# lenskit/csr

Measured on AMD Instinct MI355X. Metric: spmv_gflops, higher is better.
Workload: dtype f64

## Files before the change

### csr_amd/csrc/acc_groups.h

```cpp
#pragma once
#include <algorithm>
#include <cstdint>
#include <numeric>
#include <vector>

namespace csrk {
namespace accgroups {

constexpr int MAX_GROUPS = 3;
constexpr int XCDS = 8;

struct Deal {
    std::vector<std::vector<int32_t>> groups;
    std::vector<int32_t> first;
};

inline Deal deal_rows(const int64_t *lens, int32_t n, int G, int32_t cap)
{
    Deal d;
    d.first.push_back(0);
    if (n <= 0) return d;
    if (cap < 1) cap = 1;
    if (G < 1) G = 1;
    if (G > MAX_GROUPS) G = MAX_GROUPS;
    if (G == 1) {
        for (int32_t g0 = 0; g0 < n; g0 += cap) {
            const int32_t g1 = n - g0 < cap ? n : g0 + cap;
            std::vector<int32_t> g((size_t)(g1 - g0));
            std::iota(g.begin(), g.end(), g0);
            d.groups.push_back(std::move(g));
            d.first.push_back((int32_t)d.groups.size());
        }
        return d;
    }
    std::vector<int32_t> rank((size_t)n);
    std::iota(rank.begin(), rank.end(), 0);
    std::stable_sort(rank.begin(), rank.end(), [&](int32_t a, int32_t b) { return lens[a] > lens[b]; });
    const int64_t per_launch = (int64_t)G * cap;
    for (int64_t r0 = 0; r0 < n; r0 += per_launch) {
        const int64_t nl = n - r0 < per_launch ? n - r0 : per_launch;
        const int gb = (int)std::min<int64_t>(G, (nl + cap - 1) / cap);
        const size_t base = d.groups.size();
        d.groups.resize(base + (size_t)gb);
        for (int64_t i = 0; i < nl; i++) d.groups[base + (size_t)(i % gb)].push_back(rank[(size_t)(r0 + i)]);
        for (int g = 0; g < gb; g++) std::sort(d.groups[base + (size_t)g].begin(), d.groups[base + (size_t)g].end());
        d.first.push_back((int32_t)d.groups.size());
    }
    return d;
}

constexpr int64_t TILE_ENTRIES = 512;
constexpr int64_t MIN_SEG_TILES = 48;
inline int choose_groups(const int64_t *lens, int32_t n, int g_max, int32_t cap, int64_t floor_len, int64_t nb, int32_t cus)
{
    if (cap < 1) cap = 1;
    if (g_max > MAX_GROUPS) g_max = MAX_GROUPS;
    if (g_max < 2 || n <= cap) return 1;
    std::vector<int64_t> sl;
    for (int32_t i = 0; i < n; i++)
        if (lens[i] >= floor_len) sl.push_back(lens[i]);
    for (int g = g_max; g > 1; g--) {
        const int64_t k = std::min<int64_t>((int64_t)sl.size(), (int64_t)g * cap);
        if (k <= (int64_t)(g - 1) * cap) continue;
        if (k < (int64_t)sl.size()) std::nth_element(sl.begin(), sl.begin() + k, sl.end(), [](int64_t a, int64_t b) { return a > b; });
        int64_t entries = 0;
        for (int64_t i = 0; i < k; i++) entries += sl[(size_t)i];
        if (entries / TILE_ENTRIES >= MIN_SEG_TILES * ((int64_t)g * nb + cus)) return g;
    }
    return 1;
}

constexpr int64_t NIB_MIN_WG_TILES = 16;
inline bool choose_nib(int knob, int64_t launch_entries, int32_t launch_wgs)
{
    if (knob >= 0) return knob != 0;
    if (launch_wgs < 1) launch_wgs = 1;
    return launch_entries >= 0 && launch_entries / TILE_ENTRIES >= NIB_MIN_WG_TILES * (int64_t)launch_wgs;
}

inline int32_t group_wgs(int32_t cus, int gb, int g)
{
    const int32_t n = cus / gb + (g < cus % gb ? 1 : 0);
    return n < 1 ? 1 : n;
}

inline std::vector<uint32_t> place_wgs(const int32_t *n_wg, int gb)
{
    int64_t total = 0;
    int32_t w_max = 0;
    for (int g = 0; g < gb; g++) {
        total += n_wg[g];
        w_max = std::max(w_max, n_wg[g]);
    }
    std::vector<uint32_t> map((size_t)total, ~0u);
    int64_t fill[XCDS], room[XCDS];
    for (int c = 0; c < XCDS; c++) {
        fill[c] = 0;
        room[c] = total / XCDS + (c < total % XCDS ? 1 : 0);
    }
    std::vector<uint32_t> late;
    for (int32_t w = 0; w < w_max; w++)
        for (int g = 0; g < gb; g++) {
            if (w >= n_wg[g]) continue;
            const uint32_t id = ((uint32_t)g << 16) | (uint32_t)w;
            const int c = w % XCDS;
            if (fill[c] < room[c]) map[(size_t)(c + XCDS * fill[c]++)] = id;
            else late.push_back(id);
        }
    size_t b = 0;
    for (uint32_t id : late) {
        while (map[b] != ~0u) b++;
        map[b] = id;
    }
    return map;
}

}
}
```

### csr_amd/csrc/spmv_plan.hip

```cpp
#include "spmv_plan.h"

#include <algorithm>
#include <cstring>
#include <ctime>
#include <type_traits>

namespace csrk {
struct PlanTrace {
    bool on;
    double t0;
    static double now()
    {
        timespec ts;
        clock_gettime(CLOCK_MONOTONIC, &ts);
        return ts.tv_sec * 1e3 + ts.tv_nsec * 1e-6;
    }
    PlanTrace() : on(getenv("CSRK_PLAN_TRACE") != nullptr), t0(0.0)
    {
        if (on) {
            (void)hipDeviceSynchronize();
            t0 = now();
        }
    }
    void lap(const char *what)
    {
        if (!on) return;
        (void)hipDeviceSynchronize();
        const double t = now();
        fprintf(stderr, "[csrk plan] %-28s %8.3f ms\n", what, t - t0);
        t0 = t;
    }
};

template <class P>
__global__ void merge_plan_kernel(const P *__restrict__ rp, int32_t nrows, int64_t nnz, int items,
                                  int64_t n_tiles, int32_t *__restrict__ tile_row)
{
    int64_t t = (int64_t)blockIdx.x * blockDim.x + threadIdx.x;
    if (t > n_tiles) return;
    int64_t total = (int64_t)nrows + nnz;
    int64_t d = t * items;
    if (d > total) d = total;
    int64_t lo = d - nnz > 0 ? d - nnz : 0;
    int64_t hi = d < nrows ? d : nrows;
    while (lo < hi) {
        int64_t mid = (lo + hi) >> 1;
        if ((int64_t)rp[mid + 1] <= d - mid - 1)
            lo = mid + 1;
        else
            hi = mid;
    }
    tile_row[t] = (int32_t)lo;
}

constexpr int HOT_TABLE = 8192, HOT_PROBE = 4;
constexpr int HOT_THREADS = 512;
template <class P>
__global__ __launch_bounds__(HOT_THREADS) void hot_count_kernel(const P *__restrict__ rp, const P *__restrict__ rp_light,
                                                               const int32_t *__restrict__ ci, int32_t nrows, int64_t row_stride,
                                                               int32_t *__restrict__ cnt, unsigned long long *__restrict__ total)
{
    __shared__ int32_t s_key[HOT_TABLE];
    __shared__ int32_t s_cnt[HOT_TABLE];
    __shared__ int32_t s_start[HOT_THREADS / WAVE][WAVE];
    for (int k = threadIdx.x; k < HOT_TABLE; k += HOT_THREADS) {
        s_key[k] = -1;
        s_cnt[k] = 0;
    }
    __syncthreads();
    const int lane = threadIdx.x & (WAVE - 1), wv = threadIdx.x / WAVE;
    int32_t *starts = s_start[wv];
    const int64_t n_groups = ((int64_t)nrows + WAVE * row_stride - 1) / (WAVE * row_stride);
    unsigned long long n = 0;
    for (int64_t q = (int64_t)blockIdx.x * (HOT_THREADS / WAVE) + wv; q < n_groups; q += (int64_t)gridDim.x * (HOT_THREADS / WAVE)) {
        const int64_t r = q * WAVE * row_stride + lane;
        int64_t s = 0;
        int32_t len = 0;
        if (r < nrows && !(rp_light && rp_light[r + 1] == rp_light[r])) {
            s = rp[r];
            const int64_t l = (int64_t)rp[r + 1] - s;
            len = (int32_t)(l > 128 ? 128 : l);
        }
        const int32_t start = wave_exscan_i32(len, lane);
        const int32_t all = __builtin_amdgcn_readlane(start + len, WAVE - 1);
        __builtin_amdgcn_wave_barrier();
        starts[lane] = start;
        __builtin_amdgcn_wave_barrier();
        for (int32_t d0 = 0; d0 < all; d0 += WAVE) {
            const int32_t d = d0 + lane;
            const bool in = d < all;
            int p = 0;
#pragma unroll
            for (int step = WAVE / 2; step; step >>= 1)
                if (in && starts[p + step] <= d) p += step;
            const int64_t k = __shfl(s, p, WAVE) + (d - __shfl(start, p, WAVE));
            if (!in) continue;
            const int32_t c = ci[k];
            uint32_t slot = ((uint32_t)c * 2654435761u) >> 19;
            bool done = false;
#pragma unroll
            for (int pr = 0; pr < HOT_PROBE && !done; pr++) {
                const int32_t old = atomicCAS(&s_key[slot], -1, c);
                if (old == -1 || old == c) {
                    atomicAdd(&s_cnt[slot], 1);
                    done = true;
                }
                slot = (slot + 1) & (HOT_TABLE - 1);
            }
            if (!done) atomicAdd(&cnt[c], 1);
        }
        if (lane == 0) n += (unsigned long long)all;
    }
    __syncthreads();
    for (int k = threadIdx.x; k < HOT_TABLE; k += HOT_THREADS)
        if (s_key[k] >= 0) atomicAdd(&cnt[s_key[k]], s_cnt[k]);
    for (int off = WAVE / 2; off; off >>= 1) n += __shfl_down(n, off, WAVE);
    if ((threadIdx.x & (WAVE - 1)) == 0 && n) atomicAdd(total, n);
}

__global__ __launch_bounds__(256) void hot_census_kernel(const int32_t *__restrict__ cnt, int32_t ncols, int32_t thr,
                                                        unsigned long long *__restrict__ out)
{
    unsigned long long n = 0, sum = 0;
    for (int64_t c = (int64_t)blockIdx.x * 256 + threadIdx.x; c < ncols; c += (int64_t)gridDim.x * 256) {
        const int32_t v = cnt[c];
        if (v >= thr) {
            n++;
            sum += (unsigned long long)v;
        }
    }
    for (int off = WAVE / 2; off; off >>= 1) {
        n += __shfl_down(n, off, WAVE);
        sum += __shfl_down(sum, off, WAVE);
    }
    if ((threadIdx.x & (WAVE - 1)) == 0 && n) {
        atomicAdd(&out[0], n);
        atomicAdd(&out[1], sum);
    }
}

constexpr int HOT_HIST = 65536, HOT_HIST_LDS = 2048;
__global__ __launch_bounds__(256) void hot_hist_kernel(const int32_t *__restrict__ cnt, int32_t ncols,
                                                      unsigned long long *__restrict__ hist_n,
                                                      unsigned long long *__restrict__ hist_sum)
{
    __shared__ unsigned int s_n[HOT_HIST_LDS];
    for (int k = threadIdx.x; k < HOT_HIST_LDS; k += 256) s_n[k] = 0u;
    __syncthreads();
    for (int64_t c = (int64_t)blockIdx.x * 256 + threadIdx.x; c < ncols; c += (int64_t)gridDim.x * 256) {
        const int32_t v = cnt[c];
        if (v < HOT_HIST_LDS) {
            atomicAdd(&s_n[v], 1u);
        } else {
            const int b = v < HOT_HIST ? v : HOT_HIST;
            atomicAdd(&hist_n[b], 1ull);
            atomicAdd(&hist_sum[b], (unsigned long long)v);
        }
// ... 635 lines not shown

__global__ void vec_fill_kernel(const int64_t *__restrict__ seg_off, int32_t nrows, int32_t *__restrict__ seg_row)
{
    int64_t r = (int64_t)blockIdx.x * blockDim.x + threadIdx.x;
    if (r >= nrows) return;
    for (int64_t q = seg_off[r]; q < seg_off[r + 1]; q++) seg_row[q] = (int32_t)r;
}

constexpr int HEAVY_STREAMS = 8;

template <class P, int VT>
static int build_panel(Matrix *m, Panel *pn, const std::vector<int32_t> &rows, int64_t nnz_rows, int32_t cb,
                       int tpw, bool xcd_streams, hipStream_t s)
{
    PlanTrace tr;
    const P *rp = (const P *)m->d_rowptrs;
    const int32_t n = (int32_t)rows.size();
    const int32_t nb = (int32_t)ceil_div(m->ncols > 0 ? m->ncols : 1, cb);
    const int64_t pairs = (int64_t)n * nb;
    CSRK_TRY(pn->row_list.alloc((size_t)n * 4));
    CSRK_TRY(stage_h2d(pn->row_list.p, rows.data(), (size_t)n * 4, s));
    DevBuf off, bends;
    CSRK_TRY(off.alloc((size_t)(pairs + 1) * 8));
    const unsigned g = (unsigned)xcd_block_chunk_grid(ceil_div(n, 256), nb);
    panel_count_kernel<P><<<g, 256, 0, s>>>(rp, m->d_colinds, pn->row_list.as<int32_t>(), n, nb, cb, off.as<int64_t>());
    CSRK_LAUNCH_CHECK();
    CSRK_TRY(exclusive_scan_i64(off.as<int64_t>(), off.as<int64_t>(), pairs, s));
    pn->p64 = nnz_rows > INT32_MAX;
    CSRK_TRY(pn->rp.alloc((size_t)(pairs + 1) * (pn->p64 ? 8 : 4)));
    CSRK_TRY(pn->ci.alloc((size_t)nnz_rows * 4));
    CSRK_TRY(pn->vs.alloc((size_t)nnz_rows * 8));
    if (pn->p64)
        panel_fill_kernel<P, VT, int64_t><<<g, 256, 0, s>>>(rp, m->d_colinds, m->d_values, pn->row_list.as<int32_t>(), n, nb,
                                                          cb, off.as<int64_t>(), pn->rp.as<int64_t>(),
                                                          pn->ci.as<int32_t>(), pn->vs.as<double>());
    else
        panel_fill_kernel<P, VT, int32_t><<<g, 256, 0, s>>>(rp, m->d_colinds, m->d_values, pn->row_list.as<int32_t>(), n, nb,
                                                          cb, off.as<int64_t>(), pn->rp.as<int32_t>(),
                                                          pn->ci.as<int32_t>(), pn->vs.as<double>());
    CSRK_LAUNCH_CHECK();
    CSRK_TRY(bends.alloc((size_t)(nb + 1) * 8));
    panel_blockends_kernel<<<(unsigned)ceil_div(nb + 1, 256), 256, 0, s>>>(off.as<int64_t>(), n, nb, bends.as<int64_t>());
    CSRK_LAUNCH_CHECK();
    std::vector<int64_t> be((size_t)nb + 1), t0((size_t)nb + 1);
    CSRK_TRY(stage_d2h(be.data(), bends.p, (size_t)(nb + 1) * 8, s));
    CSRK_HIP(hipStreamSynchronize(s));
    t0[0] = 0;
    for (int32_t b = 0; b < nb; b++) t0[b + 1] = t0[b] + ceil_div((int64_t)n + be[b + 1] - be[b], MERGE_ITEMS);
    const int64_t n_tiles = t0[nb];
    CSRK_TRY(stage_h2d(bends.p, t0.data(), (size_t)(nb + 1) * 8, s));
    tr.lap("  tier 1: count, scan, fill");
    CSRK_TRY(pn->tile.alloc((size_t)n_tiles * sizeof(PanelTile)));
    if (pn->p64)
        panel_plan_kernel<int64_t><<<(unsigned)ceil_div(n_tiles, 256), 256, 0, s>>>(
            pn->rp.as<int64_t>(), n, nb, bends.as<int64_t>(), n_tiles, MERGE_ITEMS, pn->tile.as<PanelTile>());
    else
        panel_plan_kernel<int32_t><<<(unsigned)ceil_div(n_tiles, 256), 256, 0, s>>>(
            pn->rp.as<int32_t>(), n, nb, bends.as<int64_t>(), n_tiles, MERGE_ITEMS, pn->tile.as<PanelTile>());
    CSRK_LAUNCH_CHECK();
    CSRK_REQUIRE(((int64_t)cb << PANEL_POS_BITS) <= (1ll << 32), "column block too wide for the tile's index word");
    if (n_tiles > 0) {
        panel_colsort_kernel<<<(unsigned)n_tiles, 256, 0, s>>>(pn->tile.as<PanelTile>(), cb, pn->ci.as<int32_t>(), pn->vs.as<double>());
        CSRK_LAUNCH_CHECK();
    }
    tr.lap("  tier 1: tiles, column order");

    std::vector<PanelGroup> groups;
    auto block_groups = [&](int32_t b, std::vector<PanelGroup> &out) {
        for (int64_t t = t0[b]; t < t0[b + 1]; t += tpw) {
            PanelGroup gq;
            gq.t0 = t;
            gq.nt = (int32_t)(t0[b + 1] - t < tpw ? t0[b + 1] - t : tpw);
            gq.blk = b;
            out.push_back(gq);
        }
    };
    if (!xcd_streams || nb < 2 * HEAVY_STREAMS) {
        for (int32_t b = 0; b < nb; b++) block_groups(b, groups);
    } else {
        std::vector<PanelGroup> st[HEAVY_STREAMS];
        size_t longest = 0;
        for (int32_t b = 0; b < nb; b++) block_groups(b, st[b % HEAVY_STREAMS]);
        for (int q = 0; q < HEAVY_STREAMS; q++) longest = st[q].size() > longest ? st[q].size() : longest;
        PanelGroup pad;
        pad.t0 = 0;
        pad.nt = 0;
        pad.blk = 0;
        groups.reserve(longest * HEAVY_STREAMS);
        for (size_t i = 0; i < longest; i++)
            for (int q = 0; q < HEAVY_STREAMS; q++) groups.push_back(i < st[q].size() ? st[q][i] : pad);
    }
    int32_t ncs = 0;
    {
        std::vector<PanelTile> ht((size_t)n_tiles);
        CSRK_TRY(stage_d2h(ht.data(), pn->tile.p, (size_t)n_tiles * sizeof(PanelTile), nullptr));
        std::vector<int32_t> cnt((size_t)n, 0);
        for (int64_t t = 0; t < n_tiles; t++)
            if ((int64_t)ht[(size_t)t].i1 < pairs) {
                const int32_t c = ++cnt[(size_t)(ht[(size_t)t].i1 % n)];
                ncs = c > ncs ? c : ncs;
            }
        ncs = ncs < PANEL_CARRY_ROWS ? ncs : PANEL_CARRY_ROWS;
        std::vector<int32_t> crp((size_t)n + 1, 0), cidx;
        bool listed = false;
        for (int32_t h = 0; h < n; h++) {
            crp[(size_t)h + 1] = crp[(size_t)h] + (cnt[(size_t)h] > ncs ? cnt[(size_t)h] - ncs : 0);
            listed = listed || cnt[(size_t)h] > ncs;
        }
        cidx.resize((size_t)crp[(size_t)n] + 1);
        pn->listed = crp[(size_t)n];
        std::vector<int32_t> seen((size_t)n, 0);
        for (int64_t t = 0; t < n_tiles; t++) {
            PanelTile &T = ht[(size_t)t];
            T.cslot = -1;
            if ((int64_t)T.i1 >= pairs) continue;
            const int32_t h = (int32_t)(T.i1 % n), j = seen[(size_t)h]++;
            if (j < ncs) T.cslot = pairs + (int64_t)j * n + h;
            else cidx[(size_t)(crp[(size_t)h] + j - ncs)] = (int32_t)t;
        }
        CSRK_TRY(stage_h2d(pn->tile.p, ht.data(), (size_t)n_tiles * sizeof(PanelTile), nullptr));
        if (listed) {
            CSRK_TRY(pn->crp.alloc(crp.size() * 4));
            CSRK_TRY(pn->cidx.alloc(cidx.size() * 4));
            CSRK_TRY(stage_h2d(pn->crp.p, crp.data(), crp.size() * 4, nullptr));
            CSRK_TRY(stage_h2d(pn->cidx.p, cidx.data(), cidx.size() * 4, nullptr));
        }
    }
    pn->groups = (int64_t)groups.size();
    pn->pad_groups = 0;
    for (const PanelGroup &gq : groups) pn->pad_groups += gq.nt == 0;
    CSRK_TRY(pn->group.alloc(groups.size() * sizeof(PanelGroup)));
    CSRK_TRY(stage_h2d(pn->group.p, groups.data(), groups.size() * sizeof(PanelGroup), s));
    CSRK_TRY(pn->carry_row.alloc((size_t)n_tiles * 4));
    CSRK_TRY(pn->carry_val.alloc((size_t)n_tiles * 8));
    CSRK_TRY(pn->y.alloc((size_t)(pairs + (int64_t)ncs * n) * 8));
    if (ncs) {
        std::vector<double> neg0((size_t)ncs * n, -0.0);
        CSRK_TRY(stage_h2d(pn->y.as<double>() + pairs, neg0.data(), neg0.size() * 8, s));
    }
    pn->ncs = ncs;
    CSRK_HIP(hipStreamSynchronize(s));
    tr.lap("  tier 1: groups, carries (host)");
    pn->on = true;
    pn->cb = cb;
    pn->nb = nb;
    pn->nrow = n;
    pn->rows = pairs;
    pn->tiles = n_tiles;
    pn->nnz = nnz_rows;
    return CSRK_OK;
}

enum { ACC_FORM_RAW = 0, ACC_FORM_FIX56 = 1, ACC_FORM_NIB = 2 };
template <class P, int VT>
static int build_acc_panel(Matrix *m, AccPanel *ap, const int32_t *rows, const int64_t *lens, int32_t n, int64_t nnz_rows,
                           hipStream_t s, int32_t wg_want = 0, int form = ACC_FORM_FIX56)
{
    ap->fix56 = false;
    ap->nib = false;
    ap->fx_g = 0;
    const P *rp = (const P *)m->d_rowptrs;
    const int32_t nb = (int32_t)ceil_div(m->ncols > 0 ? m->ncols : 1, ACC_CB);
    PlanTrace tr;
    const int64_t pairs = (int64_t)n * nb;
    CSRK_TRY(ap->row_list.alloc((size_t)n * 4));
    CSRK_TRY(stage_h2d(ap->row_list.p, rows, (size_t)n * 4, s));
    DevBuf off, bends, pstart, d_trow, d_tpiece;
    CSRK_TRY(off.alloc((size_t)(pairs + 1) * 8));
    std::vector<int32_t> trow, tpiece;
    for (int32_t c = 0; c < n; c++)
        for (int64_t pc = 0; pc * ACC_PIECE < lens[c]; pc++) {
            trow.push_back(c);
            tpiece.push_back((int32_t)pc);
        }
    const int64_t n_tasks = (int64_t)trow.size();
    CSRK_TRY(pstart.alloc((size_t)(pairs + n) * 4));
    CSRK_TRY(d_trow.alloc((size_t)(n_tasks ? n_tasks : 1) * 4));
    CSRK_TRY(d_tpiece.alloc((size_t)(n_tasks ? n_tasks : 1) * 4));
    CSRK_TRY(stage_h2d(d_trow.p, trow.data(), (size_t)n_tasks * 4, s));
    CSRK_TRY(stage_h2d(d_tpiece.p, tpiece.data(), (size_t)n_tasks * 4, s));
    acc_pairstart_kernel<P><<<(unsigned)(ceil_div(ceil_div(n_tasks * WAVE, 256), 8) * 8), 256, 0, s>>>(
        rp, m->d_colinds, ap->row_list.as<int32_t>(), n, nb, ACC_CB, d_trow.as<int32_t>(), d_tpiece.as<int32_t>(), n_tasks,
        pstart.as<int32_t>());
    CSRK_LAUNCH_CHECK();
    tr.lap("  tier 0: pair starts");
    acc_paircount_kernel<<<(unsigned)ceil_div(pairs, 256), 256, 0, s>>>(pstart.as<int32_t>(), pairs, n, off.as<int64_t>());
    CSRK_LAUNCH_CHECK();
    DevBuf gap;
    CSRK_TRY(gap.alloc((size_t)pairs * 4));
    acc_gap_kernel<<<(unsigned)ceil_div((int64_t)nb * WAVE, 256), 256, 0, s>>>(off.as<int64_t>(), n, nb, gap.as<int32_t>());
    CSRK_LAUNCH_CHECK();
    CSRK_TRY(exclusive_scan_i64(off.as<int64_t>(), off.as<int64_t>(), pairs, s));
    CSRK_TRY(bends.alloc((size_t)(nb + 1) * 8));
    panel_blockends_kernel<<<(unsigned)ceil_div(nb + 1, 256), 256, 0, s>>>(off.as<int64_t>(), n, nb, bends.as<int64_t>());
    CSRK_LAUNCH_CHECK();
    std::vector<int64_t> be((size_t)nb + 1), t0((size_t)nb + 1);
    CSRK_TRY(stage_d2h(be.data(), bends.p, (size_t)(nb + 1) * 8, s));
    CSRK_HIP(hipStreamSynchronize(s));
    t0[0] = 0;
    for (int32_t b = 0; b < nb; b++) t0[b + 1] = t0[b] + ceil_div(be[b + 1] - be[b], ACC_TILE);
    const int64_t n_tiles = t0[nb];
    CSRK_TRY(stage_h2d(bends.p, t0.data(), (size_t)(nb + 1) * 8, s));
    tr.lap("  tier 0: counts, gaps, scan");
    int cus = 0;
    CSRK_HIP(hipDeviceGetAttribute(&cus, hipDeviceAttributeMultiprocessorCount, m->device));
    int64_t n_wg = wg_want > 0 ? wg_want : cus > 0 ? cus : 256;
    if (n_wg > n_tiles) n_wg = n_tiles;
    if (n_wg < 1) n_wg = 1;
    std::vector<int64_t> wg_t0((size_t)n_wg + 1);
    int64_t share_max = 0;
    for (int64_t w = 0; w <= n_wg; w++) wg_t0[(size_t)w] = n_tiles * w / n_wg;
    for (int64_t w = 0; w < n_wg; w++) share_max = std::max(share_max, wg_t0[(size_t)w + 1] - wg_t0[(size_t)w]);
    const int64_t n_phys = share_max * n_wg;
    DevBuf d_wg_t0;
    CSRK_TRY(d_wg_t0.alloc((size_t)(n_wg + 1) * 8));
    CSRK_TRY(stage_h2d(d_wg_t0.p, wg_t0.data(), (size_t)(n_wg + 1) * 8, s));
    ap->f32 = VT == CSRK_VAL_F32;
    DevBuf fx;
    CSRK_TRY(fx.alloc(16));
    if (VT == CSRK_VAL_F64 && n > 0 && form != ACC_FORM_RAW) {
        const char *env = getenv("CSRK_SPMV_FIX56");
        if (!(env && env[0] == '0')) {
            int32_t h[4] = {0, INT32_MAX, INT32_MIN, 0};
            CSRK_TRY(stage_h2d(fx.p, h, sizeof h, s));
            acc_range_kernel<P><<<dim3((unsigned)n, 16), 256, 0, s>>>(rp, (const double *)m->d_values, ap->row_list.as<int32_t>(),
                                                                     fx.as<int32_t>());
            CSRK_LAUNCH_CHECK();
            CSRK_TRY(stage_d2h(h, fx.p, sizeof h, s));
            CSRK_HIP(hipStreamSynchronize(s));
            fix56::Range r;
            r.bad = h[0];
            r.lo = h[1];
            r.hi = h[2];
            ap->fix56 = fix56::packable(r, ap->fx_g);
            ap->nib = ap->fix56 && form == ACC_FORM_NIB;
            tr.lap("  tier 0: value grid test");
        }
    }
    CSRK_TRY(ap->idx.alloc((size_t)n_phys * ACC_TILE * 2));
    CSRK_TRY(ap->tile_row0.alloc((size_t)(n_tiles ? n_tiles : 1) * 4));
    const int32_t fill_waves = (int32_t)ceil_div(n, WAVE);
#define ACC_FILL(SV, VERIFY)                                                                                           \
    do {                                                                                                               \
        acc_fill_kernel<P, VT, SV, VERIFY><<<(unsigned)ceil_div((int64_t)nb * fill_waves * WAVE, 256), 256, 0, s>>>(   \
            rp, m->d_colinds, m->d_values, ap->row_list.as<int32_t>(), n, nb, ACC_CB, off.as<int64_t>(),               \
            bends.as<int64_t>(), pstart.as<int32_t>(), gap.as<int32_t>(), ap->vals.as<SV>(), ap->idx.as<uint16_t>(),   \
            ap->tile_row0.as<int32_t>(), d_wg_t0.as<int64_t>(), (int32_t)n_wg, fill_waves, ap->fx_g,                   \
            fx.as<int32_t>() + 3);                                                                                     \
        CSRK_LAUNCH_CHECK();                                                                                           \
        acc_pad_kernel<SV, VERIFY><<<(unsigned)nb, 256, 0, s>>>(off.as<int64_t>(), n, nb, bends.as<int64_t>(),         \
                                                                ap->vals.as<SV>(), ap->idx.as<uint16_t>(),             \
                                                                d_wg_t0.as<int64_t>(), (int32_t)n_wg, ap->fx_g,        \
                                                                fx.as<int32_t>() + 3);                                 \
        CSRK_LAUNCH_CHECK();                                                                                           \
    } while (0)
    if (ap->fix56) {
        int32_t mismatch = 1;
        if (ap->nib) {
            CSRK_TRY(ap->vals.alloc((size_t)n_phys * fix56::nib::TILE_BYTES));
            CSRK_HIP(hipMemsetAsync(ap->vals.p, 0, (size_t)n_phys * fix56::nib::TILE_BYTES, s));
            ACC_FILL(fix56::nib::Bytes, false);
            tr.lap("  tier 0: fill (nib)");
            ACC_FILL(fix56::nib::Bytes, true);
        } else {
            CSRK_TRY(ap->vals.alloc((size_t)n_phys * fix56::TILE_BYTES));
            ACC_FILL(fix56::Packed, false);
            tr.lap("  tier 0: fill (fix56)");
            ACC_FILL(fix56::Packed, true);
        }
        CSRK_TRY(stage_d2h(&mismatch, fx.as<int32_t>() + 3, 4, s));
        CSRK_HIP(hipStreamSynchronize(s));
        tr.lap(ap->nib ? "  tier 0: verify (nib)" : "  tier 0: verify (fix56)");
        if (mismatch) {
            ap->fix56 = ap->nib = false;
            ap->fx_g = 0;
        }
    }
    if (!ap->fix56) {
        CSRK_TRY(ap->vals.alloc((size_t)n_phys * ACC_TILE * (ap->f32 ? 4 : 8)));
        if (ap->f32) ACC_FILL(float, false);
        else ACC_FILL(double, false);
        tr.lap("  tier 0: fill");
    }
#undef ACC_FILL
    std::vector<AccSeg> segs;
    std::vector<int32_t> wg_seg((size_t)n_wg + 1);
    int32_t b = 0;
    for (int64_t w = 0; w < n_wg; w++) {
        wg_seg[(size_t)w] = (int32_t)segs.size();
        int64_t t = wg_t0[(size_t)w];
        const int64_t t_end = wg_t0[(size_t)w + 1];
        while (t < t_end) {
            while (t0[b + 1] <= t) b++;
            int64_t e = t_end < t0[b + 1] ? t_end : t0[b + 1];
            if (e - t > ACC_SEG_TILES) e = t + ACC_SEG_TILES;
            AccSeg sg;
            sg.tile0 = t;
            sg.ptile0 = (t - wg_t0[(size_t)w]) * n_wg + w;
            sg.ntiles = (int32_t)(e - t);
            sg.blk = b;
            segs.push_back(sg);
            t = e;
        }
    }
    wg_seg[(size_t)n_wg] = (int32_t)segs.size();
    CSRK_TRY(ap->segs.alloc(segs.size() * sizeof(AccSeg)));
    CSRK_TRY(ap->wg_seg.alloc(wg_seg.size() * 4));
    CSRK_TRY(stage_h2d(ap->segs.p, segs.data(), segs.size() * sizeof(AccSeg), s));
    CSRK_TRY(stage_h2d(ap->wg_seg.p, wg_seg.data(), wg_seg.size() * 4, s));
    CSRK_TRY(ap->partial.alloc((size_t)n_wg * n * 8));
    CSRK_TRY(ap->z.alloc((size_t)n * 8));
    ap->lds = (size_t)(ACC_CB + 2) * 8 + (size_t)((n + 1) & ~1) * 8 + (size_t)ACC_SEG_TILES * 12;
    CSRK_TRY(spmv_kernel_attributes());
    CSRK_HIP(hipStreamSynchronize(s));
    ap->nrow = n;
    ap->nb = nb;
    ap->n_wg = (int32_t)n_wg;
    ap->tiles = n_tiles;
    ap->nnz = nnz_rows;
    ap->n_segs = (int64_t)segs.size();
    if (tr.on)
        fprintf(stderr, "[csrk plan]   tier 0 group: rows %d entries %lld workgroups %lld tiles %lld, %.1f per segment%s\n", n,
                (long long)nnz_rows, (long long)n_wg, (long long)n_tiles, segs.empty() ? 0.0 : (double)n_tiles / (double)segs.size(),
                ap->nib ? " (nib)" : ap->fix56 ? " (fix56)" : ap->f32 ? " (float32)" : " (raw)");
    tr.lap("  tier 0: segments");
    return CSRK_OK;
}

static int acc_nib_knob()
{
    const char *env = getenv("CSRK_SPMV_NIB");
    if (!env || !env[0]) return -1;
    return env[0] == '0' ? 0 : 1;
}

static int acc_groups_knob()
{
    const char *e = getenv("CSRK_ACC_GROUPS");
    const int g = e ? atoi(e) : ACC_GROUPS_DEFAULT;
    return g < 1 ? 1 : g > accgroups::MAX_GROUPS ? accgroups::MAX_GROUPS : g;
}
static int32_t acc_group_rows_knob()
{
    const char *e = getenv("CSRK_ACC_GROUP_ROWS");
    const int r = e ? atoi(e) : ACC_MAXROWS;
    return r < 1 || r > ACC_MAXROWS ? ACC_MAXROWS : r;
}


template <class P>
static int build_heavy_split(Matrix *m, SpmvPlan *p, hipStream_t s, bool allow_tier1 = true)
{
    p->n_heavy = 0;
    const char *env = getenv("CSRK_SPMV_HEAVY_SPLIT");
    if (env && env[0] == '0') return CSRK_OK;
    HEAVY_MIN = 2048;
    TIERB_MIN = TIERB_MIN_DEFAULT;
    if (const char *e = getenv("CSRK_HEAVY_MIN")) HEAVY_MIN = atoi(e) > 64 ? atoi(e) : 64;
    if (const char *e = getenv("CSRK_TIERB_MIN")) TIERB_MIN = atoi(e) >= 0 ? atoi(e) : 0;
    const bool tier1 = allow_tier1 && TIERB_MIN > 0 && TIERB_MIN < HEAVY_MIN;
    const int cut_min = tier1 ? TIERB_MIN : HEAVY_MIN;
    if (m->nrows == 0 || m->nnz < cut_min) return CSRK_OK;
    if ((int64_t)m->ncols * 8 <= (4ll << 20) && !(env && env[0] == '1')) return CSRK_OK;
    const P *rp = (const P *)m->d_rowptrs;
    const int32_t nr = m->nrows;
    const unsigned g1 = (unsigned)ceil_div((int64_t)nr + 1, 256);
    PlanTrace tr;
    DevBuf flag, hlen, bad, clen;
    CSRK_TRY(flag.alloc((size_t)(nr + 2) * 4));
    CSRK_TRY(hlen.alloc((size_t)(nr + 2) * 8));
    heavy_flag_kernel<P><<<g1, 256, 0, s>>>(rp, nr, flag.as<int32_t>(), hlen.as<int64_t>(), cut_min);
    CSRK_LAUNCH_CHECK();
    CSRK_TRY(exclusive_scan_i32(flag.as<int32_t>(), flag.as<int32_t>(), nr, s));
    CSRK_TRY(exclusive_scan_i64(hlen.as<int64_t>(), hlen.as<int64_t>(), nr, s));
    int32_t n_cut = 0;
    int64_t nnz_cut = 0;
    CSRK_TRY(stage_d2h(&n_cut, flag.as<int32_t>() + nr, 4, s));
    CSRK_TRY(stage_d2h(&nnz_cut, hlen.as<int64_t>() + nr, 8, s));
    CSRK_HIP(hipStreamSynchronize(s));
    tr.lap("  split: flags + scans");
    if (n_cut == 0) return CSRK_OK;

    CSRK_TRY(p->rp_light.alloc((size_t)(nr + 1) * sizeof(P)));
    CSRK_TRY(p->heavy_row.alloc((size_t)n_cut * 4));
    CSRK_TRY(p->cut_pos.alloc((size_t)n_cut * 8));
    CSRK_TRY(p->cut_cum.alloc((size_t)(n_cut + 1) * 8));
    CSRK_TRY(clen.alloc((size_t)n_cut * 8));
    heavy_view_kernel<P><<<g1, 256, 0, s>>>(rp, nr, flag.as<int32_t>(), hlen.as<int64_t>(), p->rp_light.as<P>(),
                                          p->heavy_row.as<int32_t>(), p->cut_pos.as<int64_t>(),
                                          p->cut_cum.as<int64_t>(), clen.as<int64_t>(), n_cut);
    CSRK_LAUNCH_CHECK();
    CSRK_TRY(bad.alloc(4));
    CSRK_HIP(hipMemsetAsync(bad.p, 0, 4, s));
    heavy_sorted_kernel<P><<<(unsigned)n_cut, 1024, 0, s>>>(rp, m->d_colinds, p->heavy_row.as<int32_t>(), n_cut,
                                                         bad.as<int32_t>());
    CSRK_LAUNCH_CHECK();
    tr.lap("  split: view + sorted kernels");
    int32_t is_bad = 0;
    std::vector<int32_t> rows((size_t)n_cut);
    std::vector<int64_t> lens((size_t)n_cut);
    CSRK_TRY(stage_d2h(&is_bad, bad.p, 4, s));
    CSRK_TRY(stage_d2h(rows.data(), p->heavy_row.p, (size_t)n_cut * 4, s));
    CSRK_TRY(stage_d2h(lens.data(), clen.p, (size_t)n_cut * 8, s));
    CSRK_HIP(hipStreamSynchronize(s));
    if (tr.on) fprintf(stderr, "[csrk plan]   n_cut %d\n", n_cut);
    tr.lap("  split: copies to the host");
    if (is_bad) return CSRK_OK;

    p->acc_groups = acc_groups_knob();
    if (!getenv("CSRK_ACC_GROUPS")) {
        int cus = 0;
        CSRK_HIP(hipDeviceGetAttribute(&cus, hipDeviceAttributeMultiprocessorCount, m->device));
        const bool extend = tier1 && !getenv("CSRK_HEAVY_MIN");
        p->acc_groups = accgroups::choose_groups(lens.data(), n_cut, ACC_GROUPS_DEFAULT, acc_group_rows_knob(),
                                                 extend ? (int64_t)std::max(ACC_FLOOR, cut_min) : (int64_t)HEAVY_MIN,
                                                 ceil_div(m->ncols > 0 ? m->ncols : 1, ACC_CB), cus > 0 ? cus : 256);
    }
    const int64_t t0_cap = (int64_t)p->acc_groups * acc_group_rows_knob();
    if (tier1 && !getenv("CSRK_HEAVY_MIN")) {
        int64_t n_min = 0;
        for (int32_t c = 0; c < n_cut; c++) n_min += lens[c] >= HEAVY_MIN;
        if (n_min < t0_cap && n_cut > n_min) {
            const size_t kth = (size_t)(n_cut < t0_cap ? n_cut : t0_cap) - 1;
            int64_t thr = -1;
            {
                constexpr int64_t HB = 1 << 16;
                std::vector<int32_t> hist((size_t)HB + 1, 0);
                for (int32_t c = 0; c < n_cut; c++) hist[(size_t)(lens[c] < HB ? lens[c] : HB)]++;
                int64_t seen = hist[(size_t)HB];
                if (seen <= (int64_t)kth)
                    for (int64_t v = HB - 1; v >= 0; v--) {
                        seen += hist[(size_t)v];
                        if (seen > (int64_t)kth) {
                            thr = v;
                            break;
                        }
                    }
            }
            if (thr < 0) {
                std::vector<int64_t> sl(lens);
                std::nth_element(sl.begin(), sl.begin() + kth, sl.end(), [](int64_t a, int64_t b) { return a > b; });
                thr = sl[kth];
            }
            int64_t n_ge = 0;
            for (int32_t c = 0; c < n_cut; c++) n_ge += lens[c] >= thr;
            if (n_ge > t0_cap) thr++;
            thr = thr < ACC_FLOOR ? ACC_FLOOR : thr;
            if (thr < HEAVY_MIN) HEAVY_MIN = (int)thr;
        }
    }
    p->heavy_min = HEAVY_MIN;
    p->tier1_min = TIERB_MIN;
    std::vector<int32_t> r0, r1;
    std::vector<int64_t> len0;
    int64_t nnz1 = 0;
    r0.reserve((size_t)n_cut);
    r1.reserve((size_t)n_cut);
    len0.reserve((size_t)n_cut);
    for (int32_t c = 0; c < n_cut; c++) {
        if (lens[c] >= HEAVY_MIN) {
            r0.push_back(rows[c]);
            len0.push_back(lens[c]);
        } else {
            r1.push_back(rows[c]);
            nnz1 += lens[c];
        }
    }
    const int64_t pair_cap = 256ll << 20;
    const int64_t pairs1 = (int64_t)r1.size() * ceil_div(m->ncols > 0 ? m->ncols : 1, PANEL_CB1);
    if (pairs1 > pair_cap && tier1) return build_heavy_split<P>(m, p, s, false);

    p->n_heavy = n_cut;
    p->nnz_light = m->nnz - nnz_cut;
    p->t0_rows = std::move(r0);
    p->t0_lens = std::move(len0);
    p->t1_rows = std::move(r1);
    p->t1_nnz = nnz1;
    tr.lap("  split: host lists");
    return CSRK_OK;
}

template <class P, int VT>
static int build_acc_groups(Matrix *m, SpmvPlan *p, hipStream_t s)
{
    const std::vector<int32_t> &r0 = p->t0_rows;
    const std::vector<int64_t> &len0 = p->t0_lens;
    if (r0.empty()) return CSRK_OK;
    const accgroups::Deal deal = accgroups::deal_rows(len0.data(), (int32_t)r0.size(), p->acc_groups, acc_group_rows_knob());
    int cus = 0;
    CSRK_HIP(hipDeviceGetAttribute(&cus, hipDeviceAttributeMultiprocessorCount, m->device));
    if (cus <= 0) cus = 256;
    std::vector<int32_t> rows;
    std::vector<int64_t> lens;
    for (size_t j = 0; j + 1 < deal.first.size(); j++) {
        const int k0 = deal.first[j], gb = deal.first[j + 1] - k0;
        const size_t a0 = p->acc.size();
        int64_t launch_entries = 0;
        for (int g = 0; g < gb; g++)
            for (int32_t pos : deal.groups[(size_t)(k0 + g)]) launch_entries += len0[(size_t)pos];
        const int packed = accgroups::choose_nib(acc_nib_knob(), launch_entries, cus) ? ACC_FORM_NIB : ACC_FORM_FIX56;
        auto build = [&](int g, int form) -> int {
            const std::vector<int32_t> &pos = deal.groups[(size_t)(k0 + g)];
            rows.resize(pos.size());
            lens.resize(pos.size());
            int64_t gn = 0;
            for (size_t i = 0; i < pos.size(); i++) {
                rows[i] = r0[(size_t)pos[i]];
                lens[i] = len0[(size_t)pos[i]];
                gn += lens[i];
            }
            return build_acc_panel<P, VT>(m, p->acc[a0 + (size_t)g], rows.data(), lens.data(), (int32_t)pos.size(), gn, s,
                                          gb > 1 ? accgroups::group_wgs(cus, gb, g) : 0, form);
        };
        bool any_raw = false;
        for (int g = 0; g < gb; g++) {
            AccPanel *ap = new (std::nothrow) AccPanel();
            CSRK_REQUIRE(ap, "out of host memory");
            p->acc.push_back(ap);
            CSRK_TRY(build(g, packed));
            any_raw = any_raw || !ap->fix56;
        }
        AccPanel *head = p->acc[a0];
        if (gb == 1) continue;
        for (int g = 0; g < gb; g++)
            if (any_raw && p->acc[a0 + (size_t)g]->fix56) CSRK_TRY(build(g, ACC_FORM_RAW));
        int32_t n_wg[accgroups::MAX_GROUPS];
        for (int g = 0; g < gb; g++) {
            n_wg[g] = p->acc[a0 + (size_t)g]->n_wg;
            p->acc[a0 + (size_t)g]->launch_groups = 0;
        }
        const std::vector<uint32_t> map = accgroups::place_wgs(n_wg, gb);
        head->launch_groups = gb;
        head->launch_wgs = (int32_t)map.size();
        CSRK_TRY(head->wg_map.alloc(map.size() * 4));
        CSRK_TRY(stage_h2d(head->wg_map.p, map.data(), map.size() * 4, s));
        CSRK_HIP(hipStreamSynchronize(s));
    }
    return CSRK_OK;
}

template <class P>
static int build_tiers(Matrix *m, SpmvPlan *p, hipStream_t s)
{
    if (!p->n_heavy) return CSRK_OK;
    const std::vector<int32_t> &r1 = p->t1_rows;
    const int64_t nnz1 = p->t1_nnz;
#define BUILD(VT)                                                                                                  \
    do {                                                                                                           \
        CSRK_TRY((build_acc_groups<P, VT>(m, p, s)));                                                              \
        if (!r1.empty()) CSRK_TRY((build_panel<P, VT>(m, &p->tier1, r1, nnz1, PANEL_CB1, 1, true, s)));            \
    } while (0)
    if (m->val_type == CSRK_VAL_F64) BUILD(CSRK_VAL_F64);
    else if (m->val_type == CSRK_VAL_F32) BUILD(CSRK_VAL_F32);
    else BUILD(CSRK_VAL_NONE);
#undef BUILD
    return CSRK_OK;
}

template <class P>
static int build_hot_cache(Matrix *m, SpmvPlan *p, hipStream_t s)
{
    p->n_hot = 0;
    const char *env = getenv("CSRK_SPMV_HOT");
    if (env && env[0] == '0') return CSRK_OK;
    const bool force = env && env[0] == '1';
    if (m->nnz < 2 || m->ncols < 1) return CSRK_OK;
    PlanTrace tr;
    int64_t HOT_SLOTS = HOT_SLOTS_MAX;
    p->hot_slots = (int32_t)HOT_SLOTS;
    if (!force && (m->nnz < (1 << 20) || (int64_t)m->ncols * 8 <= (4ll << 20))) return CSRK_OK;
    const int32_t nc = m->ncols;
    DevBuf cnt, slot, census;
    CSRK_TRY(cnt.alloc((size_t)(nc + 1) * 4));
    CSRK_TRY(slot.alloc((size_t)(nc + 2) * 4));
    CSRK_TRY(census.alloc(16));
    CSRK_HIP(hipMemsetAsync(cnt.p, 0, (size_t)(nc + 1) * 4, s));
    CSRK_HIP(hipMemsetAsync(census.p, 0, 16, s));
    const int64_t row_stride = p->nnz_light > (1ll << 25) ? p->nnz_light >> 25 : 1;
    const int64_t hc_need = ceil_div(ceil_div(m->nrows, WAVE * row_stride), HOT_THREADS / WAVE);
    hot_count_kernel<P><<<(unsigned)(hc_need < 1024 ? hc_need : 1024), HOT_THREADS, 0, s>>>(
        (const P *)m->d_rowptrs, p->n_heavy ? p->rp_light.as<P>() : (const P *)nullptr, m->d_colinds, m->nrows,
        row_stride, cnt.as<int32_t>(), census.as<unsigned long long>());
    CSRK_LAUNCH_CHECK();
    unsigned long long n_samples_u = 0;
    CSRK_TRY(stage_d2h(&n_samples_u, census.p, 8, s));
    CSRK_HIP(hipStreamSynchronize(s));
    const int64_t n_samples = (int64_t)n_samples_u;
    tr.lap("  hot: column counts");
    if (n_samples == 0) return CSRK_OK;
    auto census_at = [&](int32_t thr, unsigned long long out[2]) -> int {
        CSRK_HIP(hipMemsetAsync(census.p, 0, 16, s));
        hot_census_kernel<<<1024, 256, 0, s>>>(cnt.as<int32_t>(), nc, thr, census.as<unsigned long long>());
        CSRK_LAUNCH_CHECK();
        CSRK_TRY(stage_d2h(out, census.p, 16, s));
        CSRK_HIP(hipStreamSynchronize(s));
        return CSRK_OK;
    };
    unsigned long long c[2];
    int64_t lo = 2, hi = n_samples + 1;
    bool decided = false;
    {
        DevBuf hist;
        CSRK_TRY(hist.alloc((size_t)2 * (HOT_HIST + 1) * 8));
        CSRK_HIP(hipMemsetAsync(hist.p, 0, (size_t)2 * (HOT_HIST + 1) * 8, s));
        hot_hist_kernel<<<1024, 256, 0, s>>>(cnt.as<int32_t>(), nc, hist.as<unsigned long long>(),
                                             hist.as<unsigned long long>() + (HOT_HIST + 1));
        CSRK_LAUNCH_CHECK();
        std::vector<unsigned long long> hh((size_t)2 * (HOT_HIST + 1));
        CSRK_TRY(stage_d2h(hh.data(), hist.p, hh.size() * 8, s));
        CSRK_HIP(hipStreamSynchronize(s));
        const unsigned long long *hn = hh.data(), *hs = hh.data() + (HOT_HIST + 1);
        if (hn[HOT_HIST] <= (unsigned long long)HOT_SLOTS) {
            unsigned long long n_ge = 0, s_ge = 0;
            int64_t thr0 = HOT_HIST;
            n_ge = hn[HOT_HIST];
            s_ge = hs[HOT_HIST];
            for (int64_t v = HOT_HIST - 1; v >= 2; v--) {
                if (n_ge + hn[v] > (unsigned long long)HOT_SLOTS) break;
                n_ge += hn[v];
                s_ge += hs[v];
                thr0 = v;
            }
            lo = thr0;
            c[0] = n_ge;
            c[1] = s_ge;
            decided = true;
        }
    }
    if (!decided) CSRK_TRY(census_at((int32_t)lo, c));
    if (!decided && c[0] > (unsigned long long)HOT_SLOTS) {
        while (lo + 1 < hi) {
            const int64_t mid = lo + (hi - lo) / 2;
            CSRK_TRY(census_at((int32_t)(mid > INT32_MAX ? INT32_MAX : mid), c));
            if (c[0] <= (unsigned long long)HOT_SLOTS)
                hi = mid;
            else
                lo = mid;
        }
        CSRK_TRY(census_at((int32_t)(hi > INT32_MAX ? INT32_MAX : hi), c));
        lo = hi;
    }
    const int32_t thr = (int32_t)(lo > INT32_MAX ? INT32_MAX : lo);
    const int32_t n_hot = (int32_t)c[0];
    tr.lap("  hot: threshold");
    p->hot_cover = n_samples ? (double)c[1] / (double)n_samples : 0.0;
    if (n_hot == 0 || (!force && p->hot_cover < 0.2)) return CSRK_OK;

    const unsigned gc = (unsigned)ceil_div((int64_t)nc + 1, 256);
    hot_flag_kernel<<<gc, 256, 0, s>>>(cnt.as<int32_t>(), nc, thr, slot.as<int32_t>());
    CSRK_LAUNCH_CHECK();
    CSRK_TRY(exclusive_scan_i32(slot.as<int32_t>(), slot.as<int32_t>(), nc, s));
    CSRK_TRY(p->hot_cols.alloc((size_t)n_hot * 4));
    DevBuf hcnt;
    CSRK_TRY(hcnt.alloc((size_t)n_hot * 4));
    hot_list_kernel<<<gc, 256, 0, s>>>(cnt.as<int32_t>(), slot.as<int32_t>(), nc, thr, p->hot_cols.as<int32_t>(),
                                      hcnt.as<int32_t>());
    CSRK_LAUNCH_CHECK();
    {
        const int32_t nchunk = (int32_t)ceil_div(n_hot, HS_CHUNK);
        DevBuf k2, v2, dc;
        CSRK_TRY(k2.alloc((size_t)n_hot * 4));
        CSRK_TRY(v2.alloc((size_t)n_hot * 4));
        CSRK_TRY(dc.alloc((size_t)(256 * (int64_t)nchunk + 1) * 4));
        uint32_t *ka = hcnt.as<uint32_t>(), *kb = k2.as<uint32_t>();
        int32_t *va = p->hot_cols.as<int32_t>(), *vb = v2.as<int32_t>();
        for (int pass = 0; pass < 4; pass++) {
            hot_sort_count_kernel<<<(unsigned)nchunk, WAVE, 0, s>>>(ka, n_hot, 8 * pass, nchunk, dc.as<int32_t>());
            CSRK_LAUNCH_CHECK();
            CSRK_TRY(exclusive_scan_i32(dc.as<int32_t>(), dc.as<int32_t>(), 256 * (int64_t)nchunk, s));
            hot_sort_place_kernel<<<(unsigned)nchunk, WAVE, 0, s>>>(ka, va, n_hot, 8 * pass, nchunk, dc.as<int32_t>(), kb, vb);
            CSRK_LAUNCH_CHECK();
            std::swap(ka, kb);
            std::swap(va, vb);
// ... 520 lines not shown
```

Before: 854.5.

## Align tier-0 group workgroup tile cuts across column blocks

Splits panel building into a count phase and a build phase so that all groups in a multi-group launch can be partitioned together. Each group now gets an equal number of workgroups, and per-workgroup tile ranges are cut at the same column-block positions across groups via a shared prefix sum. The intent is that workgroups with the same index in different groups touch the same x column range at the same time, which should improve cache reuse of x and balance work. This adds host-side planning cost and can leave some workgroups with uneven or empty tile shares.

```diff
diff --git a/csr_amd/csrc/acc_groups.h b/csr_amd/csrc/acc_groups.h
--- a/csr_amd/csrc/acc_groups.h
+++ b/csr_amd/csrc/acc_groups.h
@@ -84,6 +84,41 @@
     return n < 1 ? 1 : n;
 }
 
+inline int32_t equal_wgs(int32_t cus, int gb)
+{
+    const int32_t n = cus / (gb < 1 ? 1 : gb);
+    return n < 1 ? 1 : n;
+}
+
+inline std::vector<std::vector<int64_t>> aligned_cuts(const int64_t *const *t0, int gb, int64_t nb, int32_t W)
+{
+    typedef unsigned __int128 u128;
+    if (W < 1) W = 1;
+    if (nb < 0) nb = 0;
+    std::vector<std::vector<int64_t>> cuts((size_t)(gb < 0 ? 0 : gb), std::vector<int64_t>((size_t)W + 1, 0));
+    std::vector<int64_t> sum((size_t)nb + 1, 0);
+    for (int g = 0; g < gb; g++) {
+        for (int64_t b = 0; b <= nb; b++) sum[(size_t)b] += t0[g][b];
+        cuts[(size_t)g][(size_t)W] = t0[g][nb];
+    }
+    const int64_t T = sum[(size_t)nb];
+    if (T <= 0) return cuts;
+    int64_t b = 0;
+    for (int32_t w = 1; w < W; w++) {
+        const u128 pos = (u128)w * (u128)T;
+        while ((u128)sum[(size_t)b + 1] * (u128)W <= pos) b++;
+        const u128 num = pos - (u128)sum[(size_t)b] * (u128)W;
+        const u128 den = (u128)(sum[(size_t)b + 1] - sum[(size_t)b]) * (u128)W;
+        for (int g = 0; g < gb; g++) {
+            const int64_t n = t0[g][b + 1] - t0[g][b];
+            int64_t r = (int64_t)((2 * num * (u128)n + den) / (2 * den));
+            if (r > n) r = n;
+            cuts[(size_t)g][(size_t)w] = std::max(t0[g][b] + r, cuts[(size_t)g][(size_t)w - 1]);
+        }
+    }
+    return cuts;
+}
+
 inline std::vector<uint32_t> place_wgs(const int32_t *n_wg, int gb)
 {
     int64_t total = 0;
diff --git a/csr_amd/csrc/spmv_plan.hip b/csr_amd/csrc/spmv_plan.hip
--- a/csr_amd/csrc/spmv_plan.hip
+++ b/csr_amd/csrc/spmv_plan.hip
@@ -3,6 +3,7 @@
 #include <algorithm>
 #include <cstring>
 #include <ctime>
+#include <set>
 #include <type_traits>
 
 namespace csrk {
@@ -944,9 +945,17 @@
 }
 
 enum { ACC_FORM_RAW = 0, ACC_FORM_FIX56 = 1, ACC_FORM_NIB = 2 };
-template <class P, int VT>
-static int build_acc_panel(Matrix *m, AccPanel *ap, const int32_t *rows, const int64_t *lens, int32_t n, int64_t nnz_rows,
-                           hipStream_t s, int32_t wg_want = 0, int form = ACC_FORM_FIX56)
+
+struct AccCount {
+    DevBuf off, bends, pstart, gap;
+    std::vector<int64_t> t0;
+    int32_t n = 0, nb = 0;
+    int64_t nnz_rows = 0;
+};
+
+template <class P>
+static int build_acc_count(Matrix *m, AccPanel *ap, AccCount *ac, const int32_t *rows, const int64_t *lens, int32_t n,
+                           int64_t nnz_rows, hipStream_t s)
 {
     ap->fix56 = false;
     ap->nib = false;
@@ -957,7 +966,8 @@
     const int64_t pairs = (int64_t)n * nb;
     CSRK_TRY(ap->row_list.alloc((size_t)n * 4));
     CSRK_TRY(stage_h2d(ap->row_list.p, rows, (size_t)n * 4, s));
-    DevBuf off, bends, pstart, d_trow, d_tpiece;
+    DevBuf &off = ac->off, &bends = ac->bends, &pstart = ac->pstart, &gap = ac->gap;
+    DevBuf d_trow, d_tpiece;
     CSRK_TRY(off.alloc((size_t)(pairs + 1) * 8));
     std::vector<int32_t> trow, tpiece;
     for (int32_t c = 0; c < n; c++)
@@ -978,7 +988,6 @@
     tr.lap("  tier 0: pair starts");
     acc_paircount_kernel<<<(unsigned)ceil_div(pairs, 256), 256, 0, s>>>(pstart.as<int32_t>(), pairs, n, off.as<int64_t>());
     CSRK_LAUNCH_CHECK();
-    DevBuf gap;
     CSRK_TRY(gap.alloc((size_t)pairs * 4));
     acc_gap_kernel<<<(unsigned)ceil_div((int64_t)nb * WAVE, 256), 256, 0, s>>>(off.as<int64_t>(), n, nb, gap.as<int32_t>());
     CSRK_LAUNCH_CHECK();
@@ -986,22 +995,47 @@
     CSRK_TRY(bends.alloc((size_t)(nb + 1) * 8));
     panel_blockends_kernel<<<(unsigned)ceil_div(nb + 1, 256), 256, 0, s>>>(off.as<int64_t>(), n, nb, bends.as<int64_t>());
     CSRK_LAUNCH_CHECK();
-    std::vector<int64_t> be((size_t)nb + 1), t0((size_t)nb + 1);
+    std::vector<int64_t> be((size_t)nb + 1);
+    std::vector<int64_t> &t0 = ac->t0;
+    t0.assign((size_t)nb + 1, 0);
     CSRK_TRY(stage_d2h(be.data(), bends.p, (size_t)(nb + 1) * 8, s));
     CSRK_HIP(hipStreamSynchronize(s));
-    t0[0] = 0;
     for (int32_t b = 0; b < nb; b++) t0[b + 1] = t0[b] + ceil_div(be[b + 1] - be[b], ACC_TILE);
-    const int64_t n_tiles = t0[nb];
     CSRK_TRY(stage_h2d(bends.p, t0.data(), (size_t)(nb + 1) * 8, s));
     tr.lap("  tier 0: counts, gaps, scan");
+    ac->n = n;
+    ac->nb = nb;
+    ac->nnz_rows = nnz_rows;
+    return CSRK_OK;
+}
+
+template <class P, int VT>
+static int build_acc_panel(Matrix *m, AccPanel *ap, AccCount *ac, hipStream_t s, int32_t wg_want = 0,
+                           const std::vector<int64_t> *cuts = nullptr, int form = ACC_FORM_FIX56)
+{
+    ap->fix56 = false;
+    ap->nib = false;
+    ap->fx_g = 0;
+    const P *rp = (const P *)m->d_rowptrs;
+    const int32_t n = ac->n, nb = ac->nb;
+    const int64_t nnz_rows = ac->nnz_rows;
+    const std::vector<int64_t> &t0 = ac->t0;
+    DevBuf &off = ac->off, &bends = ac->bends, &pstart = ac->pstart, &gap = ac->gap;
+    const int64_t n_tiles = t0[nb];
+    PlanTrace tr;
     int cus = 0;
     CSRK_HIP(hipDeviceGetAttribute(&cus, hipDeviceAttributeMultiprocessorCount, m->device));
     int64_t n_wg = wg_want > 0 ? wg_want : cus > 0 ? cus : 256;
-    if (n_wg > n_tiles) n_wg = n_tiles;
+    if (!cuts && n_wg > n_tiles) n_wg = n_tiles;
     if (n_wg < 1) n_wg = 1;
     std::vector<int64_t> wg_t0((size_t)n_wg + 1);
     int64_t share_max = 0;
-    for (int64_t w = 0; w <= n_wg; w++) wg_t0[(size_t)w] = n_tiles * w / n_wg;
+    if (cuts) {
+        CSRK_REQUIRE((int64_t)cuts->size() == n_wg + 1 && cuts->front() == 0 && cuts->back() == n_tiles, "tier 0: cut table");
+        wg_t0 = *cuts;
+    } else {
+        for (int64_t w = 0; w <= n_wg; w++) wg_t0[(size_t)w] = n_tiles * w / n_wg;
+    }
     for (int64_t w = 0; w < n_wg; w++) share_max = std::max(share_max, wg_t0[(size_t)w + 1] - wg_t0[(size_t)w]);
     const int64_t n_phys = share_max * n_wg;
     DevBuf d_wg_t0;
@@ -1137,6 +1171,12 @@
     const char *e = getenv("CSRK_ACC_GROUP_ROWS");
     const int r = e ? atoi(e) : ACC_MAXROWS;
     return r < 1 || r > ACC_MAXROWS ? ACC_MAXROWS : r;
+}
+static int32_t acc_wgs_knob(int32_t cus)
+{
+    const char *e = getenv("CSRK_ACC_WGS");
+    const int w = e ? atoi(e) : 0;
+    return w < 1 || w > cus ? cus : w;
 }
 
 
@@ -1282,6 +1322,7 @@
     int cus = 0;
     CSRK_HIP(hipDeviceGetAttribute(&cus, hipDeviceAttributeMultiprocessorCount, m->device));
     if (cus <= 0) cus = 256;
+    PlanTrace tr;
     std::vector<int32_t> rows;
     std::vector<int64_t> lens;
     for (size_t j = 0; j + 1 < deal.first.size(); j++) {
@@ -1291,7 +1332,11 @@
         for (int g = 0; g < gb; g++)
             for (int32_t pos : deal.groups[(size_t)(k0 + g)]) launch_entries += len0[(size_t)pos];
         const int packed = accgroups::choose_nib(acc_nib_knob(), launch_entries, cus) ? ACC_FORM_NIB : ACC_FORM_FIX56;
-        auto build = [&](int g, int form) -> int {
+        AccCount cnt[accgroups::MAX_GROUPS];
+        for (int g = 0; g < gb; g++) {
+            AccPanel *ap = new (std::nothrow) AccPanel();
+            CSRK_REQUIRE(ap, "out of host memory");
+            p->acc.push_back(ap);
             const std::vector<int32_t> &pos = deal.groups[(size_t)(k0 + g)];
             rows.resize(pos.size());
             lens.resize(pos.size());
@@ -1301,16 +1346,35 @@
                 lens[i] = len0[(size_t)pos[i]];
                 gn += lens[i];
             }
-            return build_acc_panel<P, VT>(m, p->acc[a0 + (size_t)g], rows.data(), lens.data(), (int32_t)pos.size(), gn, s,
-                                          gb > 1 ? accgroups::group_wgs(cus, gb, g) : 0, form);
+            CSRK_TRY(build_acc_count<P>(m, ap, &cnt[g], rows.data(), lens.data(), (int32_t)pos.size(), gn, s));
+        }
+        const int32_t W = gb > 1 ? accgroups::equal_wgs(acc_wgs_knob(cus), gb) : 0;
+        const int32_t nb = cnt[0].nb;
+        std::vector<std::vector<int64_t>> cuts;
+        bool aligned = gb > 1;
+        for (int g = 0; g < gb; g++) aligned = aligned && cnt[g].t0[(size_t)nb] >= W;
+        if (aligned) {
+            const int64_t *t0[accgroups::MAX_GROUPS];
+            for (int g = 0; g < gb; g++) t0[g] = cnt[g].t0.data();
+            cuts = accgroups::aligned_cuts(t0, gb, nb, W);
+            if (tr.on)
+                for (int g = 0; g < gb; g++)
+                    for (int32_t w : std::set<int32_t>{0, W / 2, W - 1}) {
+                        const std::vector<int64_t> &t = cnt[g].t0, &c = cuts[(size_t)g];
+                        const bool any = c[(size_t)w] < c[(size_t)w + 1];
+                        const long b0 = any ? (long)(std::upper_bound(t.begin(), t.end(), c[(size_t)w]) - t.begin()) - 1 : -1;
+                        const long b1 = any ? (long)(std::upper_bound(t.begin(), t.end(), c[(size_t)w + 1] - 1) - t.begin()) - 1 : -1;
+                        fprintf(stderr, "[csrk plan]   tier 0 launch %zu group %d workgroup %d of %d: tiles %lld .. %lld, blocks %ld .. %ld\n",
+                                j, g, (int)w, (int)W, (long long)c[(size_t)w], (long long)c[(size_t)w + 1], b0, b1);
+                    }
+        }
+        auto build = [&](int g, int form) -> int {
+            return build_acc_panel<P, VT>(m, p->acc[a0 + (size_t)g], &cnt[g], s, W, aligned ? &cuts[(size_t)g] : nullptr, form);
         };
         bool any_raw = false;
         for (int g = 0; g < gb; g++) {
-            AccPanel *ap = new (std::nothrow) AccPanel();
-            CSRK_REQUIRE(ap, "out of host memory");
-            p->acc.push_back(ap);
             CSRK_TRY(build(g, packed));
-            any_raw = any_raw || !ap->fix56;
+            any_raw = any_raw || !p->acc[a0 + (size_t)g]->fix56;
         }
         AccPanel *head = p->acc[a0];
         if (gb == 1) continue;
```

After: 845.7. -1.0%, worse.
